# vliu15/speech-masters-thesis

Measured on AMD Instinct MI355X. Metric: LJSpeech utterances/sec per VQ-VAE train step, higher is better.
Workload: dtype bf16

## Files before the change

### include/smt_hip.h

```cpp
#ifndef SMT_HIP_H
#define SMT_HIP_H

#include <stddef.h>
#include <stdint.h>

#ifdef __cplusplus
extern "C" {
#endif

typedef void* smt_stream_t;

enum { SMT_F32 = 0, SMT_BF16 = 1 };

const char* smt_last_error(void);
int smt_abi_version(void);

size_t smt_vq_prep_bytes(int k_bins, int dim);
int smt_vq_prepare(const float* codebook, int k_bins, int dim, void* prep, size_t prep_bytes, smt_stream_t stream);

size_t smt_vq_forward_workspace_bytes(int64_t n_rows, int k_bins, int dim);
int smt_vq_forward(const float* x, const float* codebook, void* prep, const float* row_mask,
                   int64_t n_rows, int k_bins, int dim,
                   int64_t* idx, float* min_dist, float* x_d, float* sums,
                   void* workspace, size_t workspace_bytes, smt_stream_t stream);
// ... 84 lines not shown
  int dtype;
  int batch, t_in, t_out, t_y;
  int c_in, c_out;
  int taps, stride, dilation, padding, out_stride, out_offset;
  int act_out, act_grad, site_width;
  int ld_x, ld_y, ld_res, ld_act, ld_yact;
  uint32_t drop_keys[8];
  uint32_t drop_thresh16;
  float drop_scale;
  int64_t bs_x, bs_y, bs_res, bs_act, bs_yact;
  const void* x; const void* w; const float* bias; void* y; void* y_act;
  const void* res; const void* act_grad_src;
  const int* lens_in; const int* lens_out;
  int w_swizzled;
  const void* zero_page;
  const void* x2; const void* w2;
  const float* bias2;
  const int* lens_in2;
  int c_in2, ld_x2;
  int64_t bs_x2;
  const uint32_t* drop_keys_dev;
  int drop_keys_dev_stride;
} smt_conv_desc;
int smt_conv1d_ntc(const smt_conv_desc* desc, smt_stream_t stream);
const char* smt_conv1d_kernel_name(const smt_conv_desc* desc);
int smt_conv1d_dma_plan(const smt_conv_desc* desc, int* tile_rows, int* row_classes);

size_t smt_conv1d_wgrad_workspace_bytes(const smt_conv_desc* desc);
int smt_conv1d_wgrad(const smt_conv_desc* desc, float* dweight, int64_t stride_out, int64_t stride_in,
                     int64_t stride_tap, const int* tap_map, float* dbias, void* workspace,
                     size_t workspace_bytes, smt_stream_t stream);
int smt_wgrad_reduce_defer(int on, smt_stream_t stream);
const char* smt_conv1d_wgrad_kernel_name(const smt_conv_desc* desc);

size_t smt_conv1x1_bwd_workspace_bytes(const smt_conv_desc* desc);
int smt_conv1x1_bwd(const smt_conv_desc* desc, float* dweight, int64_t stride_out, int64_t stride_in, float* dbias,
                    void* workspace, size_t workspace_bytes, smt_stream_t stream);

size_t smt_conv_k1_bwd_workspace_bytes(int batch, int t);
int smt_conv_k1_bwd(const void* dh, int64_t bs_dh, int ld_dh, const void* x, int64_t bs_x, int ld_x,
                    const void* w_packed_bwd, const void* res, int64_t bs_res, int ld_res, void* dx, int64_t bs_dx,
                    int ld_dx, const int* lens, int batch, int t, const void* zero_page, float* dweight,
                    int64_t stride_out, int64_t stride_in, float* dbias, void* workspace, size_t workspace_bytes,
                    smt_stream_t stream);

int smt_convt4s2(const void* x, int64_t bs_x, int ld_x, const void* w_packed, const float* bias, void* y, int64_t bs_y,
                 int ld_y, const int* lens_in, const int* lens_out, int batch, int t_in, int c_out, const void* zero_page,
                 smt_stream_t stream);
int smt_conv4s2(const void* x, int64_t bs_x, int ld_x, const void* w_packed, const float* bias, void* y, int64_t bs_y,
                int ld_y, const int* lens_in, const int* lens_out, int batch, int t_in, int c_in, const void* zero_page,
                smt_stream_t stream);

int smt_conv_k3gate_fwd(const void* u2, int64_t bs_u2, int ld_u2, const void* x, int64_t bs_x, int ld_x,
                        const void* w3_packed, const void* w1_packed, const float* b3, const float* b1, void* z,
                        int64_t bs_z, int ld_z, void* g, int64_t bs_g, int ld_g, const int* lens, int batch, int t,
                        const void* zero_page, smt_stream_t stream);

size_t smt_conv_gate_bwd_workspace_bytes(int batch, int t);
int smt_conv_gate_bwd(const void* dy, int64_t bs_dy, int ld_dy, const void* g, int64_t bs_g, int ld_g,
                      const void* w_packed_bwd, void* dx, int64_t bs_dx, int ld_dx, const int* lens, int batch, int t,
                      const void* zero_page, float* dweight, int64_t stride_out, int64_t stride_in, float* dbias,
                      void* workspace, size_t workspace_bytes, smt_stream_t stream);

int smt_gate_mix_fwd(const void* z, void* g, int dtype, int64_t rows, int width, int depth, int ld_z, int ld_g,
                     smt_stream_t stream);
int smt_gate_mix_bwd(const void* z, const void* dg, void* dz, int dtype, int64_t rows, int width, int depth,
// ... 234 lines not shown
```

### speech-masters-thesis_amd/csrc/conv_wgrad.hip

```cpp
#include <algorithm>
#include <cstdlib>
#include <type_traits>

#include "conv_common.h"

namespace smt {

struct WgradArgs {
  const void* x; const void* dy; float* slab;
  const int* lens_in;
  long long x_bs, dy_bs;
  int ldx, ldy;
  int B, Tin, Tout, Ty, Cin, Cout;
  int taps, stride, dil, pad, out_stride, out_offset;
  int rows_per_chunk, chunks_per_batch, nblk_ci, nblk_co, with_bias;
};

template <typename T> struct WTr;
template <> struct WTr<__bf16> {
  static constexpr int R = 128;
  static constexpr int pitch(int ch) { return ch + 32; }
};
template <> struct WTr<float> {
  static constexpr int R = 64;
// ... 369 lines not shown
          acc[j] = __builtin_amdgcn_mfma_f32_32x32x16_bf16(a, bfrag, acc[j], 0, 0, 0);
        } else if (j == ntaps && bias_plane) {
          acc[j] = __builtin_amdgcn_mfma_f32_32x32x16_bf16(a, ones, acc[j], 0, 0, 0);
        }
      }
    }
    step_end_wait<0>();
  }
  const int planes = ntaps + 1;
  float* out = p.slab + ((size_t)w.cgl * w.nblk + w.blk) * (size_t)planes * CB * CIB;
#pragma unroll
  for (int j = 0; j < NT; ++j) {
    if (j >= planes) break;
#pragma unroll
    for (int e = 0; e < 16; ++e) {
      const int row = wm * 32 + (e & 3) + 8 * (e >> 2) + 4 * hh;
      const int col = wn * 32 + r;
      out[((size_t)j * CB + row) * CIB + col] = acc[j][e];
    }
  }
}

struct ShiftArgs {
  const void* x; const void* dy; float* slab; const int* lens_in;
  long long x_bs, dy_bs;
  int ldx, ldy;
  int B, Tin, Tout, pad, rs;
  int tiles_per_item, tiles_per_wg, n_chunks, nblk_ci, nblk_co, with_bias;
};

constexpr int SH_R = 128, SH_XROWS = SH_R + 8, SH_DY = SH_R * 128, SH_X = SH_XROWS * 256, SH_STAGE = SH_DY + SH_X;

template <int NTAPS>
__global__ __launch_bounds__(512) void conv_wgrad_shift_kernel(ShiftArgs p, const __bf16* __restrict__ zero_page) {
  constexpr int CB = 64, CIB = 128, WNC = 4, DYB = CB * 2, XB = CIB * 2, PLANES = NTAPS + 1;
  extern __shared__ __attribute__((aligned(16))) unsigned char smem[];
  const int tid = threadIdx.x, lane = tid & 63;
  const int wave = __builtin_amdgcn_readfirstlane(tid >> 6);
  const int wm = wave / WNC, wn = wave % WNC;
  const int r = lane & 31, hh = lane >> 5;

  const WgBlock w = wgrad_block(p.nblk_ci, p.nblk_co);
  if (w.cgl >= p.n_chunks) return;
  const int co0 = (w.blk / p.nblk_ci) * CB, ci0 = (w.blk % p.nblk_ci) * CIB;
  const int ntiles = p.tiles_per_item * p.B * p.rs;
  const int tile_begin = w.cgl * p.tiles_per_wg;
  const int tile_end = min(ntiles, tile_begin + p.tiles_per_wg);
  const int rs = p.rs;
  const bool bias_plane = p.with_bias && (ci0 == 0);

  f32x16 acc[PLANES];
#pragma unroll
  for (int j = 0; j < PLANES; ++j)
#pragma unroll
    for (int e = 0; e < 16; ++e) acc[j][e] = 0.f;

  constexpr int SH_PIECES = 7;
  constexpr int SH_PPS = 2;
  static_assert(SH_PPS <= NTAPS && SH_PPS * (SH_R / 16) >= SH_PIECES, "the pieces fit the k-loop");
  const unsigned pdy = (unsigned)p.ldy * rs * 2u, pxx = (unsigned)p.ldx * rs * 2u;
  const int dyrow = 8 * wave + (lane >> 3), xrow = 4 * wave + (lane >> 4);
  const unsigned voff_dy = (unsigned)dyrow * pdy + (unsigned)(((lane & 7) ^ swz_dy(dyrow)) << 4);
  const unsigned voff_x = (unsigned)xrow * pxx + (unsigned)(((lane & 15) ^ swz_x(xrow)) << 4);
  const unsigned voff_x6 = (128 + xrow < SH_R + NTAPS - 1) ? voff_x + 128u * pxx : 0x80000000u;
  struct Src { __amdgpu_buffer_rsrc_t rdy, rxx; unsigned sdy, sx; };
  auto item_source = [&](int item, Src& s) {
    const int b = item / rs, cls = item - b * rs;
    const int Tc = (p.Tout - cls + rs - 1) / rs;
    const int len_full = p.lens_in ? min(scalar_load_i32(p.lens_in + b), p.Tin) : p.Tin;
    const int len_in = max(0, (len_full - cls + rs - 1) / rs);
    s.rdy = ws_rsrc(p.dy, ((long long)b * p.dy_bs + (long long)cls * p.ldy + co0) * 2, (unsigned)Tc * pdy);
    s.rxx = ws_rsrc(p.x, ((long long)b * p.x_bs + (long long)cls * p.ldx + ci0) * 2, (unsigned)len_in * pxx);
  };
  auto tile_source = [&](int t0, Src& s) {
    s.sdy = (unsigned)t0 * pdy;
    s.sx = (unsigned)(t0 - p.pad) * pxx;
// ... 75 lines not shown
        const int m = s >> 1;
        u32x4 bw;
        if (s & 1) {
#pragma unroll
          for (int i = 0; i < 4; ++i) bw[i] = __builtin_amdgcn_alignbit(w[m + i + 1], w[m + i], 16);
        } else {
          bw = u32x4{w[m], w[m + 1], w[m + 2], w[m + 3]};
        }
        acc[s] = __builtin_amdgcn_mfma_f32_32x32x16_bf16(a, __builtin_bit_cast(bf16x8, bw), acc[s], 0, 0, 0);
        if (s < SH_PPS && SH_PPS * k0 + s < SH_PIECES) {
          __builtin_amdgcn_sched_barrier(0);
          piece(sn, SH_PPS * k0 + s, buf ^ 1);
          __builtin_amdgcn_sched_barrier(0);
        }
      }
      if (bias_plane && (k0 & 3) == wn) acc[NTAPS] = __builtin_amdgcn_mfma_f32_32x32x16_bf16(a, ones, acc[NTAPS], 0, 0, 0);
    }
    WG_T(c3);
    WG_ACC(0, c0, c1); WG_ACC(1, c1, c2); WG_ACC(2, c2, c3); WG_ACC(4, c0, c0 + 1);
  }
  vm_wait<0>();
  WG_T(c4);
  float* out = p.slab + ((size_t)w.cgl * w.nblk + w.blk) * (size_t)PLANES * CB * CIB;
#pragma unroll
  for (int j = 0; j < PLANES; ++j)
#pragma unroll
    for (int e = 0; e < 16; ++e) {
      const int row = wm * 32 + (e & 3) + 8 * (e >> 2) + 4 * hh;
      out[((size_t)j * CB + row) * CIB + wn * 32 + r] = acc[j][e];
    }
  WG_T(c5);
  WG_ACC(3, c4, c5);
  WG_DUMP;
}

struct ShiftPlan { int rs, pad, tiles_per_item, tiles_per_wg, n_chunks, nblk_co, nblk_ci; };
static bool wgrad_shift_plan(const smt_conv_desc* d, ShiftPlan* pl) {
  static const bool off = getenv("SMT_WGRAD_NO_SHIFT") != nullptr;
  if (off || d->dtype != SMT_BF16 || d->stride != 1 || d->out_stride != 1 || d->out_offset != 0 || !d->zero_page ||
      d->c_in % 128 != 0 || d->c_out % 64 != 0 || d->taps < 3 || d->taps > 9 || !(d->taps & 1) || d->t_in != d->t_out)
    return false;
  int rs = 1, pad = d->padding;
  if (d->dilation > 1) {
    if (d->padding % d->dilation != 0 || d->t_out / d->dilation < class_min_rows()) return false;
    rs = d->dilation; pad = d->padding / d->dilation;
  }
  if (pad < 0 || pad > d->taps - 1) return false;
  const long long tc_max = (d->t_out + rs - 1) / rs;
  const long long span = (tc_max + 2 * SH_R) * rs * 2;
  if (span * d->ld_x >= (1ll << 31) || span * d->ld_y >= (1ll << 31)) return false;
  const int tpi = (int)((tc_max + SH_R - 1) / SH_R);
  const long long ntiles = (long long)tpi * d->batch * rs;
  static const int min_tiles = getenv("SMT_SHIFT_MIN_TILES") ? atoi(getenv("SMT_SHIFT_MIN_TILES")) : 256;
  if (ntiles < min_tiles) return false;
  const int nco = d->c_out / 64, nci = d->c_in / 128;
  static const int min_tpw = getenv("SMT_SHIFT_MIN_TPW") ? atoi(getenv("SMT_SHIFT_MIN_TPW")) : 2;
  const long long chunks_target =
      std::max<long long>(8, std::min<long long>(256 / (nco * nci), ntiles / std::max(1, min_tpw)));
  const int tpw = (int)((ntiles + chunks_target - 1) / chunks_target);
  pl->rs = rs; pl->pad = pad; pl->tiles_per_item = tpi; pl->tiles_per_wg = tpw;
  pl->n_chunks = (int)((ntiles + tpw - 1) / tpw); pl->nblk_co = nco; pl->nblk_ci = nci;
  return true;
}

struct WreduceJob {
  const float* slab; float* dw; float* db;
// ... 189 lines not shown
    l = wgrad_group_plan(d, j0, std::min(WG_GROUP, d->taps - j0));
    l.ws_off = groups_ws;
    groups_ws += l.ws_bytes;
  }
  pl->ws_bytes = groups_ws;
  if (wgrad_shift_plan(d, &pl->sh)) {
    WgradLaunch l = {};
    l.variant = WG_SHIFT; l.taps = d->taps; l.pad = pl->sh.pad; l.cib = 128;
    l.n_chunks = pl->sh.n_chunks; l.nblk_co = pl->sh.nblk_co; l.nblk_ci = pl->sh.nblk_ci;
    l.grid = wgrad_grid(l); l.lds = 2 * SH_STAGE;
    l.ws_bytes = wgrad_slab_bytes(l);
    pl->n = 1; pl->l[0] = l;
    pl->ws_bytes = std::max(l.ws_bytes, groups_ws);
  }
  return true;
}

extern "C" size_t smt_conv1d_wgrad_workspace_bytes(const smt_conv_desc* d) {
  WgradPlan pl;
  return wgrad_plan(d, &pl) ? pl.ws_bytes : 0;
}

extern "C" const char* smt_conv1d_wgrad_kernel_name(const smt_conv_desc* d) {
  WgradPlan pl;
  return wgrad_plan(d, &pl) ? kWgradName[pl.l[0].variant] : "";
}

template <typename... P, typename... A>
static void launch_lds(void (*kernel)(P...), unsigned grid, unsigned threads, size_t lds, hipStream_t stream, A... args) {
  (void)hipFuncSetAttribute((const void*)kernel, hipFuncAttributeMaxDynamicSharedMemorySize, (int)WG_MAX_LDS);
  kernel<<<dim3(grid), dim3(threads), lds, stream>>>(args...);
}

typedef void (*WgradKernel)(WgradArgs);
static_assert(WG_GROUP == 5, "the kernels are instantiated for 2 .. 6 accumulator planes (1 .. 5 taps + bias)");
#define SMT_WG_BY_PLANES(planes, K) \
  ((planes) == 2 ? K(2) : (planes) == 3 ? K(3) : (planes) == 4 ? K(4) : (planes) == 5 ? K(5) : K(6))
template <typename T, int CIB, bool STRIDED> static WgradKernel generic_kernel(int planes) {
#define SMT_WG_K(NT) (WgradKernel)conv_wgrad_kernel<T, NT, CIB, STRIDED>
  return SMT_WG_BY_PLANES(planes, SMT_WG_K);
#undef SMT_WG_K
}
static WgradKernel dma_kernel(int planes) {
#define SMT_WG_K(NT) (WgradKernel)conv_wgrad_dma_kernel<NT>
  return SMT_WG_BY_PLANES(planes, SMT_WG_K);
#undef SMT_WG_K
}

extern "C" int smt_conv1d_wgrad(const smt_conv_desc* d, float* dweight, int64_t stride_out, int64_t stride_in,
                                int64_t stride_tap, const int* tap_map, float* dbias, void* workspace,
                                size_t workspace_bytes, smt_stream_t stream_) {
  hipStream_t stream = (hipStream_t)stream_;
  SMT_CHECK_ARG(d && tap_map, "smt_conv1d_wgrad: null pointer");
  SMT_CHECK_ARG(d->taps >= 1 && d->taps <= WG_MAX_TAPS, "smt_conv1d_wgrad: taps must be in [1, 16]");
  SMT_CHECK_ARG(d->x && d->y && dweight && workspace, "smt_conv1d_wgrad: null pointer");
  SMT_CHECK_ARG(d->dtype == SMT_BF16 || d->dtype == SMT_F32, "smt_conv1d_wgrad: bad dtype");
  const bool bf = d->dtype == SMT_BF16;
  const int epv = bf ? 8 : 4;
  SMT_CHECK_ARG(d->c_in % epv == 0 && d->c_out % epv == 0 && d->ld_x % epv == 0 && d->ld_y % epv == 0,
                "smt_conv1d_wgrad: channels / pitches must keep 16-byte alignment");
  WgradPlan pl;
  wgrad_plan(d, &pl);
  SMT_CHECK_ARG(workspace_bytes >= pl.ws_bytes, "smt_conv1d_wgrad: workspace too small");
  const bool empty = d->batch <= 0 || d->t_out <= 0;
  for (int i = 0; i < pl.n; ++i) {
    const WgradLaunch& l = pl.l[i];
    float* slab = reinterpret_cast<float*>((char*)workspace + l.ws_off);
    float* db = i == 0 ? dbias : nullptr;
    if (l.variant == WG_SHIFT) {
      ShiftArgs a;
      a.x = d->x; a.dy = d->y; a.slab = slab; a.lens_in = d->lens_in;
      a.x_bs = d->bs_x; a.dy_bs = d->bs_y; a.ldx = d->ld_x; a.ldy = d->ld_y;
      a.B = d->batch; a.Tin = d->t_in; a.Tout = d->t_out; a.pad = l.pad; a.rs = pl.sh.rs;
      a.tiles_per_item = pl.sh.tiles_per_item; a.tiles_per_wg = pl.sh.tiles_per_wg; a.n_chunks = l.n_chunks;
      a.nblk_ci = l.nblk_ci; a.nblk_co = l.nblk_co; a.with_bias = db ? 1 : 0;
      const __bf16* zp = (const __bf16*)d->zero_page;
      switch (d->taps) {
        case 3: launch_lds(conv_wgrad_shift_kernel<3>, l.grid, 512, l.lds, stream, a, zp); break;
        case 5: launch_lds(conv_wgrad_shift_kernel<5>, l.grid, 512, l.lds, stream, a, zp); break;
        case 7: launch_lds(conv_wgrad_shift_kernel<7>, l.grid, 512, l.lds, stream, a, zp); break;
        default: launch_lds(conv_wgrad_shift_kernel<9>, l.grid, 512, l.lds, stream, a, zp); break;
      }
      SMT_CHECK_LAUNCH(kWgradName[l.variant]);
    } else if (!empty) {
      SMT_CHECK_ARG(l.lds <= WG_MAX_LDS, "conv_wgrad: tile needs %zu B of LDS", l.lds);
      WgradArgs a;
      a.x = d->x; a.dy = d->y; a.slab = slab; a.lens_in = d->lens_in;
      a.x_bs = d->bs_x; a.dy_bs = d->bs_y; a.ldx = d->ld_x; a.ldy = d->ld_y;
      a.B = d->batch; a.Tin = d->t_in; a.Tout = d->t_out; a.Ty = d->t_y; a.Cin = d->c_in; a.Cout = d->c_out;
      a.taps = l.taps; a.stride = d->stride; a.dil = d->dilation; a.pad = l.pad;
      a.out_stride = d->out_stride; a.out_offset = d->out_offset;
      a.rows_per_chunk = l.rows_per_chunk; a.chunks_per_batch = l.chunks_per_batch;
      a.nblk_ci = l.nblk_ci; a.nblk_co = l.nblk_co; a.with_bias = db ? 1 : 0;
      const bool strided = d->stride > 1;
      const int planes = l.taps + 1;
      const WgradKernel k = l.variant == WG_DMA ? dma_kernel(planes)
                          : bf && l.cib == 128  ? generic_kernel<__bf16, 128, false>(planes)
                          : bf ? (strided ? generic_kernel<__bf16, 64, true>(planes) : generic_kernel<__bf16, 64, false>(planes))
                               : (strided ? generic_kernel<float, 64, true>(planes) : generic_kernel<float, 64, false>(planes));
      launch_lds(k, l.grid, l.variant == WG_DMA ? 512 : l.cib * 4, l.lds, stream, a);
      SMT_CHECK_LAUNCH(kWgradName[l.variant]);
    }
    const int bias_cols = l.variant == WG_SHIFT ? 4 : 1;
    int rc = launch_wgrad_reduce(slab, dweight, db, empty ? 0 : l.n_chunks, l.nblk_co, l.nblk_ci, l.taps, d->c_in, d->c_out,
                                 l.cib, stride_out, stride_in, stride_tap, tap_map + l.j0, stream, bias_cols);
    if (rc) return rc;
  }
  return 0;
}
```

### speech-masters-thesis_amd/smt_amd/convops.py

```python
import contextlib
import ctypes
import os
from dataclasses import dataclass

import torch

from . import native as N
from . import packing
from . import profiler
from .packing import Part

SMT_F32, SMT_BF16 = 0, 1
_DT = {torch.float32: SMT_F32, torch.bfloat16: SMT_BF16}


class ConvDesc(ctypes.Structure):
    _fields_ = [("dtype", ctypes.c_int), ("batch", ctypes.c_int), ("t_in", ctypes.c_int), ("t_out", ctypes.c_int),
                ("t_y", ctypes.c_int), ("c_in", ctypes.c_int), ("c_out", ctypes.c_int), ("taps", ctypes.c_int),
                ("stride", ctypes.c_int), ("dilation", ctypes.c_int), ("padding", ctypes.c_int),
                ("out_stride", ctypes.c_int), ("out_offset", ctypes.c_int), ("act_out", ctypes.c_int),
                ("act_grad", ctypes.c_int), ("site_width", ctypes.c_int), ("ld_x", ctypes.c_int),
                ("ld_y", ctypes.c_int), ("ld_res", ctypes.c_int), ("ld_act", ctypes.c_int), ("ld_yact", ctypes.c_int),
                ("drop_keys", ctypes.c_uint32 * 8), ("drop_thresh16", ctypes.c_uint32), ("drop_scale", ctypes.c_float),
                ("bs_x", ctypes.c_int64), ("bs_y", ctypes.c_int64), ("bs_res", ctypes.c_int64),
# ... 45 lines not shown
def _i32(lens):
    if lens is None:
        return None
    return lens if lens.dtype == torch.int32 else lens.to(torch.int32)


_zero_pages = {}


def _zero_page(device):
    key = (device.type, device.index)
    if key not in _zero_pages:
        _zero_pages[key] = torch.zeros(4096, dtype=torch.uint8, device=device)
    return _zero_pages[key]


def _dma_ok(dtype, c_in, c_out):
    return dtype == torch.bfloat16 and c_in % 128 == 0 and c_out % 128 == 0


def _phases(kernel, stride, padding):
    out = []
    for ph in range(stride):
        taps = [(j, (ph + padding - j) // stride) for j in range(kernel) if (ph + padding - j) % stride == 0]
        taps.sort(key=lambda jt: jt[1])
        offs = [o for _, o in taps]
        assert offs == list(range(offs[0], offs[0] + len(offs))), "phase taps must touch consecutive rows"
        out.append(([j for j, _ in taps], -offs[0]))
    return out


_K3GATE = not bool(int(os.environ.get("SMT_NO_K3GATE", "0")))
_RESAMPLE = not bool(int(os.environ.get("SMT_NO_RESAMPLE", "0")))
_WN_TAIL = not bool(int(os.environ.get("SMT_NO_WN_TAIL", "0")))
_WN_TAIL_WIDTHS = (64, 128)


def _pack(weight, dtype, n_out, n_in, s_out, s_in, s_tap, tap_map, swizzle=False):
    return packing.pack([Part.dense(weight, n_out, n_in, s_out, s_in, s_tap, tap_map, swizzle)], dtype,
                        (len(tap_map), n_out, n_in))


def _pack_fwd(weight, dtype, swizzle=False):
    c_out, c_in, k = weight.shape
    return _pack(weight, dtype, c_out, c_in, c_in * k, k, 1, range(k), swizzle)


def _pack_bwd(weight, dtype, swizzle=False):
    c_out, c_in, k = weight.shape
    return _pack(weight, dtype, c_in, c_out, k, c_in * k, 1, range(k - 1, -1, -1), swizzle)


def _pack_cat_fwd(weights, dtype, swizzle=False):
    n_in = weights[0].shape[1]
    total = sum(w.shape[0] for w in weights)
    parts, row0 = [], 0
    for w in weights:
        parts.append(Part(w, w.shape[0], n_in, n_in, 1, 1, (0,), bool(swizzle), row0 * n_in, total * n_in, n_in))
        row0 += w.shape[0]
    return packing.pack(parts, dtype, (1, total, n_in))


def _pack_cat_bwd(weights, dtype):
    n_in = weights[0].shape[1]
    total = sum(w.shape[0] for w in weights)
    parts, col0 = [], 0
# ... 59 lines not shown

def _conv_bytes(d, esz):
    outs = (1 if d.y else 0) + (1 if d.act_out else 0) + (1 if d.res else 0) + (1 if d.act_grad else 0)
    rows_in = float(d.batch) * d.t_in * (d.c_in + (d.c_in2 if d.x2 else 0))
    return (rows_in + float(d.batch) * d.t_out * d.c_out * outs) * esz + d.taps * d.c_in * d.c_out * esz


def _base_desc(x, y, lens_in, c_in, c_out, taps, stride, dil, pad, t_out, out_stride=1, out_offset=0, t_y=None):
    d = ConvDesc()
    d.dtype = _DT[x.dtype]
    d.batch, d.t_in, d.t_out, d.t_y = x.shape[0], x.shape[1], t_out, (y.shape[1] if t_y is None else t_y)
    d.c_in, d.c_out = c_in, c_out
    d.taps, d.stride, d.dilation, d.padding = taps, stride, dil, pad
    d.out_stride, d.out_offset = out_stride, out_offset
    d.x, d.bs_x, d.ld_x = _geom(x)
    if y is not None:
        d.y, d.bs_y, d.ld_y = _geom(y)
    d.lens_in = _p(lens_in)
    d.drop_scale = 1.0
    return d


def _wgrad(desc, dweight, s_out, s_in, s_tap, tap_map, dbias):
    lib = N.lib()
    desc.zero_page = _p(_zero_page(dweight.device))
    ws_bytes = lib.smt_conv1d_wgrad_workspace_bytes(ctypes.byref(desc))
    ws = N.workspace.get(ws_bytes, dweight.device)
    arr = (ctypes.c_int * len(tap_map))(*tap_map)
    dtype = "bf16" if desc.dtype == SMT_BF16 else "f32"
    name = lib.smt_conv1d_wgrad_kernel_name(ctypes.byref(desc)).decode() + ("_" + _tag(desc) if profiler.DETAIL else "")
    with profiler.region(name, flops=_conv_flops(desc), bound="mfma", dtype=dtype):
        N.check(lib.smt_conv1d_wgrad(ctypes.byref(desc), _p(dweight), s_out, s_in, s_tap, arr, _p(dbias), _p(ws),
                                     ws.numel(), N.stream_ptr()), "smt_conv1d_wgrad")


def _conv1x1_bwd(desc, dweight, s_out, s_in, dbias):
    lib = N.lib()
    ws_bytes = lib.smt_conv1x1_bwd_workspace_bytes(ctypes.byref(desc))
    ws = N.workspace.get(ws_bytes, dweight.device)
    rows = float(desc.batch) * desc.t_out
    name = "conv1x1_bwd" + ("_" + _tag(desc) if profiler.DETAIL else "")
    with profiler.region(name, flops=2 * _conv_flops(desc), nbytes=rows * 3 * desc.c_in * 2, bound="hbm", dtype="bf16"):
        N.check(lib.smt_conv1x1_bwd(ctypes.byref(desc), _p(dweight), s_out, s_in, _p(dbias), _p(ws), ws.numel(),
                                    N.stream_ptr()), "smt_conv1x1_bwd")


def _conv_gate_bwd(dy, g, w_packed_bwd, dx, lens32, dweight, dbias):
    lib = N.lib()
    b, t = g.shape[0], g.shape[1]
    ws = N.workspace.get(lib.smt_conv_gate_bwd_workspace_bytes(b, t), g.device)
    (pdy, bsdy, lddy), (pg, bsg, ldg), (pdx, bsdx, lddx) = _geom(dy), _geom(g), _geom(dx)
    rows = float(b) * t
    with profiler.region("conv_gate_bwd", flops=4.0 * rows * 64 * 64, nbytes=rows * 3 * 64 * 2, bound="hbm", dtype="bf16"):
        N.check(lib.smt_conv_gate_bwd(pdy, bsdy, lddy, pg, bsg, ldg, _p(w_packed_bwd), pdx, bsdx, lddx, _p(lens32), b, t,
                                      _p(_zero_page(g.device)), _p(dweight), dweight.stride(0), dweight.stride(1),
                                      _p(dbias), _p(ws), ws.numel(), N.stream_ptr()), "smt_conv_gate_bwd")


def _conv_k1_bwd(dh, x, w_packed_bwd, res, dx, lens32, dweight, dbias):
    lib = N.lib()
    b, t = x.shape[0], x.shape[1]
    ws = N.workspace.get(lib.smt_conv_k1_bwd_workspace_bytes(b, t), x.device)
    (pdh, bsdh, lddh), (px, bsx, ldx_), (pr, bsr, ldr), (pdx, bsdx, lddx) = _geom(dh), _geom(x), _geom(res), _geom(dx)
    rows = float(b) * t
    with profiler.region("conv_k1_bwd", flops=4.0 * rows * 512 * 64, nbytes=rows * (512 + 3 * 64) * 2, bound="hbm",
                         dtype="bf16"):
# ... 470 lines not shown
        geometry, scale, has_lens = ctx.cfg
        lens32 = lens32 if has_lens else None
        dout = dout.contiguous()
        with reduce_batch(x.device):
            return _GatedHiFi._backward(x, lens32, u1, u2, z, g, params, geometry, scale, dout)

    @staticmethod
    def _backward(x, lens32, u1, u2, z, g, params, geometry, scale, dout):
        depth = len(geometry)
        b, t, w = x.shape
        c2 = 2 * w
        dt, dev = x.dtype, x.device
        br = [params[6 * d:6 * d + 6] for d in range(depth)]
        wg, bg = params[6 * depth], params[6 * depth + 1]
        grads = [None] * len(params)

        def f32(shape):
            return torch.empty(shape, dtype=torch.float32, device=dev)

        dg = torch.empty_like(g)
        grads[6 * depth], grads[6 * depth + 1] = torch.empty_like(wg), f32(bg.shape)
        if dt == torch.bfloat16 and w == 64:
            _conv_gate_bwd(dout, g, _pack_bwd(wg, dt), dg, lens32, grads[6 * depth], grads[6 * depth + 1])
        else:
            d = _dgrad_stride1(dout, _pack_bwd(wg, dt), dg, 1, 1, 0)
            d.lens_out = _p(lens32)
            _launch(d, "conv_dgrad", _conv_flops(d), _conv_bytes(d, x.element_size()))
            _wgrad(_base_desc(g, dout, lens32, w, w, 1, 1, 1, 0, t), grads[6 * depth], w, 1, 1, [0], grads[6 * depth + 1])

        dz = torch.empty_like(z)
        _gate_mix_bwd(z, dg, dz, depth)
        del dg
        dh1 = torch.empty_like(z)
        dh2 = torch.empty(b, t, c2, dtype=dt, device=dev)
        for dd, (k, dil, pad) in enumerate(geometry):
            sl = slice(dd * c2, (dd + 1) * c2)
            w1, b1, w2, b2, w3, b3 = br[dd]
            dz_d, u1_d, u2_d = dz[:, :, sl], u1[:, :, sl], u2[:, :, sl]
            dma = _dma_ok(dt, c2, c2)
            wb3 = _pack_bwd(w3, dt, dma)
            d = _dgrad_stride1(dz_d, wb3, dh2, 1, 1, 0)
            if dma:
                _use_dma(d, wb3)
            _set_act_grad(d, u2_d, scale)
            grads[6 * dd + 4], grads[6 * dd + 5] = torch.empty_like(w3), f32(b3.shape)
            if dma and c2 == 128:
                _conv1x1_bwd(d, grads[6 * dd + 4], c2, 1, grads[6 * dd + 5])
            else:
                _launch(d, "conv_dgrad", _conv_flops(d), _conv_bytes(d, x.element_size()))
                _wgrad(_base_desc(u2_d, dz_d, None, c2, c2, 1, 1, 1, 0, t), grads[6 * dd + 4], c2, 1, 1, [0],
                       grads[6 * dd + 5])
            wb2 = _pack_bwd(w2, dt, dma)
            d = _dgrad_stride1(dh2, wb2, dh1[:, :, sl], k, dil, pad)
            if dma:
                _use_dma(d, wb2)
            _set_act_grad(d, u1_d, scale)
            d.res, d.bs_res, d.ld_res = _geom(dz_d)
            _launch(d, "conv_dgrad", _conv_flops(d), _conv_bytes(d, x.element_size()))
            grads[6 * dd + 2], grads[6 * dd + 3] = torch.empty_like(w2), f32(b2.shape)
            _wgrad(_base_desc(u1_d, dh2, None, c2, c2, k, 1, dil, pad, t), grads[6 * dd + 2], c2 * k, k, 1,
                   list(range(k)), grads[6 * dd + 3])
        del dz, dh2
        dx = torch.empty_like(x)
        dw1cat, db1cat = torch.empty(depth * c2, w, 1, dtype=torch.float32, device=dev), f32((depth * c2,))
        if dt == torch.bfloat16 and w == 64 and depth * c2 == 512:
            _conv_k1_bwd(dh1, x, _pack_cat_bwd([p[0] for p in br], dt), dout, dx, lens32, dw1cat, db1cat)
        else:
            d = _dgrad_stride1(dh1, _pack_cat_bwd([p[0] for p in br], dt), dx, 1, 1, 0)
            d.lens_out = _p(lens32)
            d.res, d.bs_res, d.ld_res = _geom(dout)
            _launch(d, "conv_dgrad", _conv_flops(d), _conv_bytes(d, x.element_size()))
            _wgrad(_base_desc(x, dh1, lens32, w, depth * c2, 1, 1, 1, 0, t), dw1cat, w, 1, 1, [0], db1cat)
        for dd in range(depth):
            grads[6 * dd] = dw1cat[dd * c2:(dd + 1) * c2]
            grads[6 * dd + 1] = db1cat[dd * c2:(dd + 1) * c2]
        return (dx, None, None, None, None, *grads)


def gated_hifi_block(x, lens, geometry, params, *, p_drop, training, seed, site_base):
    return _GatedHiFi.apply(x, lens, tuple(geometry), (p_drop, training, seed, site_base), len(params), *params)
```

### speech-masters-thesis_amd/smt_amd/native.py

```python
import contextlib
import ctypes
import os
import threading

import torch

_HERE = os.path.dirname(os.path.abspath(__file__))
LIB_PATH = os.environ.get("SMT_HIP_LIB") or os.path.join(_HERE, "libsmt_hip.so")
ABI_VERSION = 10

_lib = None
_lock = threading.Lock()

c_i64 = ctypes.c_int64
c_int = ctypes.c_int
c_f32 = ctypes.c_float
c_u32 = ctypes.c_uint32
c_ptr = ctypes.c_void_p
c_size = ctypes.c_size_t

_SIGNATURES = {
    "smt_last_error": (ctypes.c_char_p, []),
    "smt_abi_version": (c_int, []),
    "smt_vq_forward_workspace_bytes": (c_size, [c_i64, c_int, c_int]),
    "smt_vq_prep_bytes": (c_size, [c_int, c_int]),
    "smt_vq_prepare": (c_int, [c_ptr, c_int, c_int, c_ptr, c_size, c_ptr]),
    "smt_vq_forward": (c_int, [c_ptr, c_ptr, c_ptr, c_ptr, c_i64, c_int, c_int, c_ptr, c_ptr, c_ptr, c_ptr, c_ptr, c_size,
                               c_ptr]),
    "smt_vq_backward": (c_int, [c_ptr, c_ptr, c_ptr, c_ptr, c_ptr, c_ptr, c_i64, c_int, c_ptr, c_ptr]),
    "smt_vq_ema_accumulate_workspace_bytes": (c_size, [c_i64, c_int, c_int]),
    "smt_vq_ema_accumulate": (c_int, [c_ptr, c_ptr, c_ptr, c_i64, c_int, c_int, c_ptr, c_ptr, c_size, c_ptr]),
    "smt_vq_ema_apply": (c_int, [c_ptr, c_ptr, c_ptr, c_ptr, c_ptr, c_f32, c_f32, c_int, c_int, c_ptr, c_ptr, c_size,
                                 c_ptr]),
    "smt_vq_grouped_prep_bytes": (c_size, [c_int, c_int, c_int]),
    "smt_vq_grouped_prepare": (c_int, [c_ptr, c_int, c_int, c_int, c_ptr, c_size, c_ptr]),
    "smt_vq_align_groups": (c_int, [c_ptr, c_ptr, c_int, c_int, c_int, c_int, c_ptr, c_ptr, c_ptr]),
    "smt_vq_grouped_forward_workspace_bytes": (c_size, [c_i64]),
    "smt_vq_grouped_forward": (c_int, [c_ptr, c_ptr, c_ptr, c_ptr, c_ptr, c_i64, c_int, c_int, c_int, c_ptr, c_ptr, c_ptr, c_ptr,
                                       c_ptr, c_ptr, c_size, c_ptr]),
    "smt_vq_grouped_ema_apply": (c_int, [c_ptr, c_ptr, c_ptr, c_ptr, c_ptr, c_f32, c_f32, c_int, c_int, c_int, c_ptr, c_ptr,
                                         c_size, c_ptr]),
    "smt_pack_weight": (c_int, [c_ptr, c_ptr, c_int, c_int, c_int, c_int, c_i64, c_i64, c_i64, c_ptr, c_int, c_ptr]),
    "smt_pack_weights_batched": (c_int, [c_ptr, c_ptr, c_ptr, c_int, c_ptr]),
    "smt_conv1d_ntc": (c_int, [c_ptr, c_ptr]),
    "smt_conv1d_kernel_name": (ctypes.c_char_p, [c_ptr]),
    "smt_conv1d_dma_plan": (c_int, [c_ptr, c_ptr, c_ptr]),
    "smt_conv1d_wgrad_workspace_bytes": (c_size, [c_ptr]),
    "smt_conv1d_wgrad_kernel_name": (ctypes.c_char_p, [c_ptr]),
    "smt_conv1d_wgrad": (c_int, [c_ptr, c_ptr, c_i64, c_i64, c_i64, c_ptr, c_ptr, c_ptr, c_size, c_ptr]),
    "smt_wgrad_reduce_defer": (c_int, [c_int, c_ptr]),
    "smt_conv1x1_bwd_workspace_bytes": (c_size, [c_ptr]),
    "smt_conv1x1_bwd": (c_int, [c_ptr, c_ptr, c_i64, c_i64, c_ptr, c_ptr, c_size, c_ptr]),
    "smt_conv_gate_bwd_workspace_bytes": (c_size, [c_int, c_int]),
    "smt_conv_gate_bwd": (c_int, [c_ptr, c_i64, c_int, c_ptr, c_i64, c_int, c_ptr, c_ptr, c_i64, c_int, c_ptr, c_int,
                                  c_int, c_ptr, c_ptr, c_i64, c_i64, c_ptr, c_ptr, c_size, c_ptr]),
    "smt_conv_k1_bwd_workspace_bytes": (c_size, [c_int, c_int]),
    "smt_conv_k1_bwd": (c_int, [c_ptr, c_i64, c_int, c_ptr, c_i64, c_int, c_ptr, c_ptr, c_i64, c_int, c_ptr, c_i64,
                                c_int, c_ptr, c_int, c_int, c_ptr, c_ptr, c_i64, c_i64, c_ptr, c_ptr, c_size, c_ptr]),
    "smt_convt4s2": (c_int, [c_ptr, c_i64, c_int, c_ptr, c_ptr, c_ptr, c_i64, c_int, c_ptr, c_ptr, c_int, c_int, c_int, c_ptr, c_ptr]),
    "smt_conv4s2": (c_int, [c_ptr, c_i64, c_int, c_ptr, c_ptr, c_ptr, c_i64, c_int, c_ptr, c_ptr, c_int, c_int, c_int, c_ptr, c_ptr]),
    "smt_conv_k3gate_fwd": (c_int, [c_ptr, c_i64, c_int, c_ptr, c_i64, c_int, c_ptr, c_ptr, c_ptr, c_ptr, c_ptr, c_i64, c_int,
                                    c_ptr, c_i64, c_int, c_ptr, c_int, c_int, c_ptr, c_ptr]),
    "smt_gate_mix_fwd": (c_int, [c_ptr, c_ptr, c_int, c_i64, c_int, c_int, c_int, c_int, c_ptr]),
    "smt_gate_mix_bwd": (c_int, [c_ptr, c_ptr, c_ptr, c_int, c_i64, c_int, c_int, c_int, c_int, c_int, c_ptr]),
    "smt_wavenet_gate_fwd": (c_int, [c_ptr, c_i64, c_int, c_ptr, c_i64, c_int, c_ptr, c_int, c_int, c_int, c_int, c_ptr]),
    "smt_wavenet_gate_bwd": (c_int, [c_ptr, c_i64, c_int, c_ptr, c_i64, c_int, c_ptr, c_i64, c_int, c_ptr, c_int, c_int, c_int,
                                     c_int, c_ptr]),
    "smt_wavenet_tail_fwd": (c_int, [c_ptr, c_i64, c_int, c_ptr, c_i64, c_int, c_ptr, c_ptr, c_ptr, c_i64, c_int, c_ptr, c_int,
                                     c_int, c_int, c_ptr]),
    "smt_conv_in_fwd": (c_int, [c_ptr, c_ptr, c_ptr, c_ptr, c_ptr, c_int, c_int, c_int, c_int, c_int, c_int, c_int,
                                c_int, c_ptr]),
    "smt_conv_in_wgrad_workspace_bytes": (c_size, [c_int, c_int, c_int]),
    "smt_conv_in_wgrad": (c_int, [c_ptr, c_ptr, c_ptr, c_ptr, c_ptr, c_int, c_int, c_int, c_int, c_int, c_int, c_int,
                                  c_int, c_ptr, c_size, c_ptr]),
    "smt_conv_out_fwd": (c_int, [c_ptr, c_ptr, c_ptr, c_ptr, c_ptr, c_int, c_int, c_int, c_int, c_ptr]),
    "smt_conv_out_bwd_workspace_bytes": (c_size, [c_int, c_int, c_int]),
    "smt_maximum_path": (c_int, [c_ptr, c_ptr, c_int, c_int, c_int, c_f32, c_ptr, c_ptr]),
    "smt_vqtts_distance": (c_int, [c_ptr, c_ptr, c_ptr, c_int, c_int, c_int, c_int, c_ptr]),
    "smt_vqtts_align_workspace_bytes": (c_size, [c_int, c_int, c_int]),
    "smt_vqtts_align": (c_int, [c_ptr, c_ptr, c_ptr, c_ptr, c_int, c_int, c_int, c_int, c_ptr, c_ptr, c_ptr, c_size, c_ptr]),
    "smt_vqtts_align_loss": (c_int, [c_ptr, c_ptr, c_ptr, c_int, c_int, c_int, c_int, c_ptr, c_ptr, c_ptr]),
    "smt_vqtts_align_loss_bwd": (c_int, [c_ptr, c_ptr, c_ptr, c_ptr, c_ptr, c_int, c_int, c_int, c_int, c_ptr, c_ptr, c_ptr]),
# ... 205 lines not shown
```

Baseline: 532.2.

## Batch per-branch shift wgrad convs into one grouped multi-job kernel launch

Adds a grouped wgrad kernel that runs the shift-kernel weight gradients of 2–4 parallel conv branches in one launch. Each workgroup slot is mapped to a job, and a greedy planner splits tiles across jobs using a per-tap cost estimate so the branches finish together. The multi-branch gated block backward now keeps a separate dh2 buffer per branch so all branch wgrads can be deferred and issued together. The aim is to remove under-filled grids and tail idle time from several small sequential launches. The cost is extra dh2 memory and a runtime switch on tap count inside the kernel, which may raise register pressure.

```diff
diff --git a/include/smt_hip.h b/include/smt_hip.h
--- a/include/smt_hip.h
+++ b/include/smt_hip.h
@@ -140,6 +140,11 @@
                      size_t workspace_bytes, smt_stream_t stream);
 int smt_wgrad_reduce_defer(int on, smt_stream_t stream);
 const char* smt_conv1d_wgrad_kernel_name(const smt_conv_desc* desc);
+size_t smt_conv1d_wgrad_multi_workspace_bytes(const smt_conv_desc* descs, int n);
+int smt_conv1d_wgrad_multi_plan(const smt_conv_desc* descs, int n, int* n_chunks_out, int* tiles_per_wg_out);
+int smt_conv1d_wgrad_multi(const smt_conv_desc* descs, int n, float* const* dweight, const int64_t* stride_out,
+                           const int64_t* stride_in, const int64_t* stride_tap, const int* tap_maps, float* const* dbias,
+                           void* workspace, size_t workspace_bytes, smt_stream_t stream);
 
 size_t smt_conv1x1_bwd_workspace_bytes(const smt_conv_desc* desc);
 int smt_conv1x1_bwd(const smt_conv_desc* desc, float* dweight, int64_t stride_out, int64_t stride_in, float* dbias,
diff --git a/speech-masters-thesis_amd/csrc/conv_wgrad.hip b/speech-masters-thesis_amd/csrc/conv_wgrad.hip
--- a/speech-masters-thesis_amd/csrc/conv_wgrad.hip
+++ b/speech-masters-thesis_amd/csrc/conv_wgrad.hip
@@ -425,7 +425,7 @@
 constexpr int SH_R = 128, SH_XROWS = SH_R + 8, SH_DY = SH_R * 128, SH_X = SH_XROWS * 256, SH_STAGE = SH_DY + SH_X;
 
 template <int NTAPS>
-__global__ __launch_bounds__(512) void conv_wgrad_shift_kernel(ShiftArgs p, const __bf16* __restrict__ zero_page) {
+__device__ __forceinline__ void wgrad_shift_body(const ShiftArgs& p, const WgBlock w) {
   constexpr int CB = 64, CIB = 128, WNC = 4, DYB = CB * 2, XB = CIB * 2, PLANES = NTAPS + 1;
   extern __shared__ __attribute__((aligned(16))) unsigned char smem[];
   const int tid = threadIdx.x, lane = tid & 63;
@@ -433,8 +433,6 @@
   const int wm = wave / WNC, wn = wave % WNC;
   const int r = lane & 31, hh = lane >> 5;
 
-  const WgBlock w = wgrad_block(p.nblk_ci, p.nblk_co);
-  if (w.cgl >= p.n_chunks) return;
   const int co0 = (w.blk / p.nblk_ci) * CB, ci0 = (w.blk % p.nblk_ci) * CIB;
   const int ntiles = p.tiles_per_item * p.B * p.rs;
   const int tile_begin = w.cgl * p.tiles_per_wg;
@@ -576,6 +574,37 @@
   WG_T(c5);
   WG_ACC(3, c4, c5);
   WG_DUMP;
+}
+
+template <int NTAPS>
+__global__ __launch_bounds__(512) void conv_wgrad_shift_kernel(ShiftArgs p, const __bf16* __restrict__ zero_page) {
+  const WgBlock w = wgrad_block(p.nblk_ci, p.nblk_co);
+  if (w.cgl >= p.n_chunks) return;
+  wgrad_shift_body<NTAPS>(p, w);
+}
+
+constexpr int SHM_MAXJ = 4;
+struct ShiftMulti { ShiftArgs job[SHM_MAXJ]; int taps[SHM_MAXJ]; int first[SHM_MAXJ + 1]; int nblk; };
+
+__global__ __launch_bounds__(512) void conv_wgrad_shift_multi_kernel(ShiftMulti m, const __bf16* __restrict__ zero_page) {
+  WgBlock w;
+  const int xcd = blockIdx.x & 7, q = blockIdx.x >> 3;
+  w.nblk = m.nblk;
+  w.blk = q % m.nblk;
+  const int slot = (q / m.nblk) * 8 + xcd;
+  if (slot >= m.first[SHM_MAXJ]) return;
+  int k = 0;
+#pragma unroll
+  for (int i = 1; i < SHM_MAXJ; ++i)
+    if (slot >= m.first[i]) k = i;
+  w.cgl = slot - m.first[k];
+  const ShiftArgs p = m.job[k];
+  switch (m.taps[k]) {
+    case 3: wgrad_shift_body<3>(p, w); break;
+    case 5: wgrad_shift_body<5>(p, w); break;
+    case 7: wgrad_shift_body<7>(p, w); break;
+    default: wgrad_shift_body<9>(p, w); break;
+  }
 }
 
 struct ShiftPlan { int rs, pad, tiles_per_item, tiles_per_wg, n_chunks, nblk_co, nblk_ci; };
@@ -831,6 +860,16 @@
   kernel<<<dim3(grid), dim3(threads), lds, stream>>>(args...);
 }
 
+static ShiftArgs shift_args(const smt_conv_desc* d, const ShiftPlan& sh, float* slab, bool with_bias) {
+  ShiftArgs a;
+  a.x = d->x; a.dy = d->y; a.slab = slab; a.lens_in = d->lens_in;
+  a.x_bs = d->bs_x; a.dy_bs = d->bs_y; a.ldx = d->ld_x; a.ldy = d->ld_y;
+  a.B = d->batch; a.Tin = d->t_in; a.Tout = d->t_out; a.pad = sh.pad; a.rs = sh.rs;
+  a.tiles_per_item = sh.tiles_per_item; a.tiles_per_wg = sh.tiles_per_wg; a.n_chunks = sh.n_chunks;
+  a.nblk_ci = sh.nblk_ci; a.nblk_co = sh.nblk_co; a.with_bias = with_bias ? 1 : 0;
+  return a;
+}
+
 typedef void (*WgradKernel)(WgradArgs);
 static_assert(WG_GROUP == 5, "the kernels are instantiated for 2 .. 6 accumulator planes (1 .. 5 taps + bias)");
 #define SMT_WG_BY_PLANES(planes, K) \
@@ -867,12 +906,7 @@
     float* slab = reinterpret_cast<float*>((char*)workspace + l.ws_off);
     float* db = i == 0 ? dbias : nullptr;
     if (l.variant == WG_SHIFT) {
-      ShiftArgs a;
-      a.x = d->x; a.dy = d->y; a.slab = slab; a.lens_in = d->lens_in;
-      a.x_bs = d->bs_x; a.dy_bs = d->bs_y; a.ldx = d->ld_x; a.ldy = d->ld_y;
-      a.B = d->batch; a.Tin = d->t_in; a.Tout = d->t_out; a.pad = l.pad; a.rs = pl.sh.rs;
-      a.tiles_per_item = pl.sh.tiles_per_item; a.tiles_per_wg = pl.sh.tiles_per_wg; a.n_chunks = l.n_chunks;
-      a.nblk_ci = l.nblk_ci; a.nblk_co = l.nblk_co; a.with_bias = db ? 1 : 0;
+      const ShiftArgs a = shift_args(d, pl.sh, slab, db != nullptr);
       const __bf16* zp = (const __bf16*)d->zero_page;
       switch (d->taps) {
         case 3: launch_lds(conv_wgrad_shift_kernel<3>, l.grid, 512, l.lds, stream, a, zp); break;
@@ -907,3 +941,113 @@
   }
   return 0;
 }
+
+static int shift_tile_cost(int taps) { return taps <= 3 ? 2892 : taps <= 5 ? 3622 : taps <= 7 ? 4686 : 5856; }
+
+struct ShiftMultiPlan {
+  int n, nblk;
+  ShiftPlan sh[SHM_MAXJ];
+  int first[SHM_MAXJ + 1];
+  unsigned grid;
+  size_t ws_off[SHM_MAXJ], ws_bytes;
+};
+
+static bool shift_multi_shares_override(int n, const long long* ntiles, long long* share) {
+  const char* s = getenv("SMT_WGRAD_MULTI_SHARES");
+  if (!s || !*s) return false;
+  for (int k = 0; k < n; ++k) {
+    char* end = nullptr;
+    share[k] = strtoll(s, &end, 10);
+    if (end == s || share[k] < 1 || share[k] > ntiles[k] || *end != (k + 1 < n ? ',' : '\0')) { share[0] = -1; return true; }
+    s = end + 1;
+  }
+  return true;
+}
+
+static bool wgrad_shift_multi_plan(const smt_conv_desc* descs, int n, ShiftMultiPlan* mp) {
+  if (!descs || n < 2 || n > SHM_MAXJ) return false;
+  long long ntiles[SHM_MAXJ], share[SHM_MAXJ];
+  for (int k = 0; k < n; ++k) {
+    if (!wgrad_shift_plan(&descs[k], &mp->sh[k])) return false;
+    const ShiftPlan& s = mp->sh[k];
+    if (s.nblk_co * s.nblk_ci != mp->sh[0].nblk_co * mp->sh[0].nblk_ci) return false;
+    ntiles[k] = (long long)s.tiles_per_item * descs[k].batch * s.rs;
+  }
+  mp->n = n; mp->nblk = mp->sh[0].nblk_co * mp->sh[0].nblk_ci;
+  if (shift_multi_shares_override(n, ntiles, share)) {
+    if (share[0] < 0) return false;
+  } else {
+    const int slots = 256 / mp->nblk;
+    if (slots < n) return false;
+    auto finish = [&](int k) { return (ntiles[k] + share[k] - 1) / share[k] * shift_tile_cost(descs[k].taps); };
+    for (int k = 0; k < n; ++k) share[k] = 1;
+    for (int given = n; given < slots; ++given) {
+      int last = -1;
+      for (int k = 0; k < n; ++k)
+        if (share[k] < ntiles[k] && (last < 0 || finish(k) > finish(last))) last = k;
+      if (last < 0) break;
+      share[last] += 1;
+    }
+  }
+  size_t off = 0;
+  mp->first[0] = 0;
+  for (int k = 0; k < n; ++k) {
+    ShiftPlan& s = mp->sh[k];
+    s.tiles_per_wg = (int)((ntiles[k] + share[k] - 1) / share[k]);
+    s.n_chunks = (int)((ntiles[k] + s.tiles_per_wg - 1) / s.tiles_per_wg);
+    mp->first[k + 1] = mp->first[k] + s.n_chunks;
+    mp->ws_off[k] = off;
+    off += align_up((size_t)s.n_chunks * mp->nblk * (descs[k].taps + 1) * 64 * 128 * sizeof(float), 256);
+  }
+  for (int k = n; k < SHM_MAXJ; ++k) mp->first[k + 1] = mp->first[n];
+  mp->ws_bytes = off;
+  mp->grid = (unsigned)(8 * ((mp->first[n] + 7) / 8) * mp->nblk);
+  return true;
+}
+
+extern "C" size_t smt_conv1d_wgrad_multi_workspace_bytes(const smt_conv_desc* descs, int n) {
+  ShiftMultiPlan mp;
+  return wgrad_shift_multi_plan(descs, n, &mp) ? mp.ws_bytes : 0;
+}
+
+extern "C" int smt_conv1d_wgrad_multi_plan(const smt_conv_desc* descs, int n, int* n_chunks_out, int* tiles_per_wg_out) {
+  ShiftMultiPlan mp;
+  if (!wgrad_shift_multi_plan(descs, n, &mp)) return 0;
+  for (int k = 0; k < n; ++k) {
+    if (n_chunks_out) n_chunks_out[k] = mp.sh[k].n_chunks;
+    if (tiles_per_wg_out) tiles_per_wg_out[k] = mp.sh[k].tiles_per_wg;
+  }
+  return n;
+}
+
+extern "C" int smt_conv1d_wgrad_multi(const smt_conv_desc* descs, int n, float* const* dweight, const int64_t* stride_out,
+                                      const int64_t* stride_in, const int64_t* stride_tap, const int* tap_maps,
+                                      float* const* dbias, void* workspace, size_t workspace_bytes, smt_stream_t stream_) {
+  hipStream_t stream = (hipStream_t)stream_;
+  SMT_CHECK_ARG(descs && dweight && stride_out && stride_in && stride_tap && tap_maps && dbias && workspace,
+                "smt_conv1d_wgrad_multi: null pointer");
+  ShiftMultiPlan mp;
+  SMT_CHECK_ARG(wgrad_shift_multi_plan(descs, n, &mp),
+                "smt_conv1d_wgrad_multi: not 2 .. 4 convs of the shift kernel (smt_conv1d_wgrad_multi_workspace_bytes returns 0)");
+  SMT_CHECK_ARG(workspace_bytes >= mp.ws_bytes, "smt_conv1d_wgrad_multi: workspace too small");
+  ShiftMulti m = {};
+  for (int k = 0; k < n; ++k) {
+    SMT_CHECK_ARG(descs[k].x && descs[k].y && dweight[k], "smt_conv1d_wgrad_multi: null pointer");
+    float* slab = reinterpret_cast<float*>((char*)workspace + mp.ws_off[k]);
+    m.job[k] = shift_args(&descs[k], mp.sh[k], slab, dbias[k] != nullptr);
+    m.taps[k] = descs[k].taps;
+  }
+  for (int k = n; k < SHM_MAXJ; ++k) { m.job[k] = m.job[0]; m.taps[k] = m.taps[0]; }
+  for (int k = 0; k <= SHM_MAXJ; ++k) m.first[k] = mp.first[k];
+  m.nblk = mp.nblk;
+  launch_lds(conv_wgrad_shift_multi_kernel, mp.grid, 512, (size_t)2 * SH_STAGE, stream, m, (const __bf16*)descs[0].zero_page);
+  SMT_CHECK_LAUNCH("conv_wgrad_shift_multi");
+  for (int k = 0; k < n; ++k) {
+    const ShiftPlan& s = mp.sh[k];
+    int rc = launch_wgrad_reduce(m.job[k].slab, dweight[k], dbias[k], s.n_chunks, s.nblk_co, s.nblk_ci, descs[k].taps,
+                                 descs[k].c_in, descs[k].c_out, 128, stride_out[k], stride_in[k], stride_tap[k],
+                                 tap_maps + k * WG_MAX_TAPS, stream, 4);
+    if (rc) return rc;
+  }
+  return 0;
+}
diff --git a/speech-masters-thesis_amd/smt_amd/convops.py b/speech-masters-thesis_amd/smt_amd/convops.py
--- a/speech-masters-thesis_amd/smt_amd/convops.py
+++ b/speech-masters-thesis_amd/smt_amd/convops.py
@@ -101,6 +101,7 @@
 
 _K3GATE = not bool(int(os.environ.get("SMT_NO_K3GATE", "0")))
 _RESAMPLE = not bool(int(os.environ.get("SMT_NO_RESAMPLE", "0")))
+_WGRAD_MULTI = not bool(int(os.environ.get("SMT_NO_WGRAD_MULTI", "0")))
 _WN_TAIL = not bool(int(os.environ.get("SMT_NO_WN_TAIL", "0")))
 _WN_TAIL_WIDTHS = (64, 128)
 
@@ -226,6 +227,33 @@
     with profiler.region(name, flops=_conv_flops(desc), bound="mfma", dtype=dtype):
         N.check(lib.smt_conv1d_wgrad(ctypes.byref(desc), _p(dweight), s_out, s_in, s_tap, arr, _p(dbias), _p(ws),
                                      ws.numel(), N.stream_ptr()), "smt_conv1d_wgrad")
+
+
+def _wgrad_multi(jobs):
+    lib = N.lib()
+    n = len(jobs)
+    dev = jobs[0][1].device
+    descs = (ConvDesc * n)()
+    for i, job in enumerate(jobs):
+        descs[i] = job[0]
+        descs[i].zero_page = _p(_zero_page(dev))
+    ws_bytes = lib.smt_conv1d_wgrad_multi_workspace_bytes(descs, n) if _WGRAD_MULTI and 2 <= n <= 4 else 0
+    if ws_bytes == 0:
+        for job in jobs:
+            _wgrad(*job)
+        return
+    ws = N.workspace.get(ws_bytes, dev)
+    ptrs = lambda ts: (ctypes.c_void_p * n)(*[None if t is None else t.data_ptr() for t in ts])
+    i64s = lambda vs: (ctypes.c_int64 * n)(*vs)
+    maps = (ctypes.c_int * (16 * n))()
+    for i, job in enumerate(jobs):
+        maps[16 * i:16 * i + len(job[5])] = job[5]
+    name = "conv_wgrad_shift" + ("_multi" + str(n) if profiler.DETAIL else "")
+    with profiler.region(name, flops=sum(_conv_flops(job[0]) for job in jobs), bound="mfma", dtype="bf16"):
+        N.check(lib.smt_conv1d_wgrad_multi(descs, n, ptrs([j[1] for j in jobs]), i64s([j[2] for j in jobs]),
+                                           i64s([j[3] for j in jobs]), i64s([j[4] for j in jobs]), maps,
+                                           ptrs([j[6] for j in jobs]), _p(ws), ws.numel(), N.stream_ptr()),
+                "smt_conv1d_wgrad_multi")
 
 
 def _conv1x1_bwd(desc, dweight, s_out, s_in, dbias):
@@ -762,8 +790,11 @@
         _gate_mix_bwd(z, dg, dz, depth)
         del dg
         dh1 = torch.empty_like(z)
-        dh2 = torch.empty(b, t, c2, dtype=dt, device=dev)
+        multi = _WGRAD_MULTI and dt == torch.bfloat16 and 2 <= depth <= 4
+        dh2_all = torch.empty(depth if multi else 1, b, t, c2, dtype=dt, device=dev)
+        k2_jobs = []
         for dd, (k, dil, pad) in enumerate(geometry):
+            dh2 = dh2_all[dd if multi else 0]
             sl = slice(dd * c2, (dd + 1) * c2)
             w1, b1, w2, b2, w3, b3 = br[dd]
             dz_d, u1_d, u2_d = dz[:, :, sl], u1[:, :, sl], u2[:, :, sl]
@@ -788,9 +819,13 @@
             d.res, d.bs_res, d.ld_res = _geom(dz_d)
             _launch(d, "conv_dgrad", _conv_flops(d), _conv_bytes(d, x.element_size()))
             grads[6 * dd + 2], grads[6 * dd + 3] = torch.empty_like(w2), f32(b2.shape)
-            _wgrad(_base_desc(u1_d, dh2, None, c2, c2, k, 1, dil, pad, t), grads[6 * dd + 2], c2 * k, k, 1,
-                   list(range(k)), grads[6 * dd + 3])
-        del dz, dh2
+            k2_jobs.append((_base_desc(u1_d, dh2, None, c2, c2, k, 1, dil, pad, t), grads[6 * dd + 2], c2 * k, k, 1,
+                            list(range(k)), grads[6 * dd + 3]))
+            if not multi:
+                _wgrad(*k2_jobs.pop())
+        if k2_jobs:
+            _wgrad_multi(k2_jobs)
+        del dz, dh2, dh2_all
         dx = torch.empty_like(x)
         dw1cat, db1cat = torch.empty(depth * c2, w, 1, dtype=torch.float32, device=dev), f32((depth * c2,))
         if dt == torch.bfloat16 and w == 64 and depth * c2 == 512:
diff --git a/speech-masters-thesis_amd/smt_amd/native.py b/speech-masters-thesis_amd/smt_amd/native.py
--- a/speech-masters-thesis_amd/smt_amd/native.py
+++ b/speech-masters-thesis_amd/smt_amd/native.py
@@ -48,6 +48,9 @@
     "smt_conv1d_wgrad_workspace_bytes": (c_size, [c_ptr]),
     "smt_conv1d_wgrad_kernel_name": (ctypes.c_char_p, [c_ptr]),
     "smt_conv1d_wgrad": (c_int, [c_ptr, c_ptr, c_i64, c_i64, c_i64, c_ptr, c_ptr, c_ptr, c_size, c_ptr]),
+    "smt_conv1d_wgrad_multi_workspace_bytes": (c_size, [c_ptr, c_int]),
+    "smt_conv1d_wgrad_multi_plan": (c_int, [c_ptr, c_int, c_ptr, c_ptr]),
+    "smt_conv1d_wgrad_multi": (c_int, [c_ptr, c_int, c_ptr, c_ptr, c_ptr, c_ptr, c_ptr, c_ptr, c_ptr, c_size, c_ptr]),
     "smt_wgrad_reduce_defer": (c_int, [c_int, c_ptr]),
     "smt_conv1x1_bwd_workspace_bytes": (c_size, [c_ptr]),
     "smt_conv1x1_bwd": (c_int, [c_ptr, c_ptr, c_i64, c_i64, c_ptr, c_ptr, c_size, c_ptr]),
```

Result: no change. 534.6 (median of 5 runs) (+0.5%).
